# 34j/vr180-convert

Hardware: NVIDIA B200
Metric: SBS equirect output Mpix/s (higher is better)
Workload: dtype f64 coordinates / u8 fixed-point (INTER_BITS=5) sampling

## Files before the change

### vr180-convert_b200/csrc/api.cu

```cuda
#include <algorithm>
#include <mutex>
#include <new>
#include <string>
#include <vector>

#include "common.cuh"

namespace vr180 {

std::atomic<uint64_t> g_launches{0};
std::atomic<int> g_debug_frames_per_cta{0};
std::atomic<int> g_debug_tiled_flags{-1};
std::atomic<int> g_debug_max_frames_per_cta{0};
std::atomic<int> g_debug_stream_grid{0};
static thread_local std::string t_cuda_error;

void set_cuda_error(cudaError_t e, const char* where) {
    t_cuda_error = std::string(cudaGetErrorName(e)) + ": " + cudaGetErrorString(e) + " at " + where;
    cudaGetLastError();
}

const std::vector<int16_t>& host_table(int K);

}

using namespace vr180;

extern "C" {

int vr180_abi_version(void) { return VR180_ABI_VERSION; }

const char* vr180_status_string(int status) {
    switch (status) {
        case VR180_OK: return "ok";
        case VR180_ERR_INVALID_ARG: return "invalid argument";
        case VR180_ERR_UNSUPPORTED: return "unsupported configuration";
        case VR180_ERR_CUDA: return "CUDA error";
        case VR180_ERR_NO_DEVICE: return "no CUDA device";
        case VR180_ERR_CHAIN: return "malformed chain descriptor";
        case VR180_ERR_NOMEM: return "out of memory";
        default: return "unknown status";
    }
}

const char* vr180_last_cuda_error(void) { return t_cuda_error.c_str(); }

int vr180_device_info(int device, char* name, size_t name_len, int* sm_count, int* cc_major, int* cc_minor) {
    int n = 0;
    if (cudaGetDeviceCount(&n) != cudaSuccess) {
        cudaGetLastError();
        return 0;
    }
    if (device >= 0 && device < n) {
        cudaDeviceProp prop;
        if (cudaGetDeviceProperties(&prop, device) == cudaSuccess) {
            if (name && name_len) {
                strncpy(name, prop.name, name_len - 1);
                name[name_len - 1] = 0;
            }
            if (sm_count) *sm_count = prop.multiProcessorCount;
            if (cc_major) *cc_major = prop.major;
            if (cc_minor) *cc_minor = prop.minor;
        }
    }
    return n;
}

uint64_t vr180_launch_count(void) { return g_launches.load(std::memory_order_relaxed); }

int vr180_debug_weight_table(int K, int16_t* out) {
    if ((K != 4 && K != 8) || !out) return VR180_ERR_INVALID_ARG;
    const auto& t = host_table(K);
    memcpy(out, t.data(), t.size() * sizeof(int16_t));
    return VR180_OK;
}

int vr180_debug_set(int what, int value) {
    if (what == 0) return g_debug_frames_per_cta.exchange(value < 0 ? 0 : value);
    if (what == 1) return g_debug_tiled_flags.exchange(value);
    if (what == 2) return g_debug_max_frames_per_cta.exchange(value < 0 ? 0 : value);
    if (what == 3) return g_debug_stream_grid.exchange(value < 0 ? 0 : value);
    return VR180_ERR_INVALID_ARG;
}

int vr180_build_map(const vr180_chain_t* chain, int out_w, int out_h, float* xmap_dev, float* ymap_dev,
                    int64_t map_pitch, void* stream) {
    if (!chain || !xmap_dev || !ymap_dev || out_w <= 0 || out_h <= 0 || map_pitch < out_w) return VR180_ERR_INVALID_ARG;
    const int rc = validate_chain(chain);
    if (rc != VR180_OK) return rc;
    DeviceGuard g(xmap_dev);
    if (!g.ok) return VR180_ERR_INVALID_ARG;
    return launch_build_map(chain, out_w, out_h, xmap_dev, ymap_dev, map_pitch, (cudaStream_t)stream);
}

int vr180_pack_lut(const float* xmap_dev, const float* ymap_dev, int64_t map_pitch, int out_w, int out_h,
                   int32_t* fixed_dev, int64_t fixed_pitch, void* stream) {
    if (!xmap_dev || !ymap_dev || !fixed_dev || out_w <= 0 || out_h <= 0 || map_pitch < out_w || fixed_pitch < out_w)
        return VR180_ERR_INVALID_ARG;
    DeviceGuard g(fixed_dev);
    if (!g.ok) return VR180_ERR_INVALID_ARG;
    return launch_pack_lut(xmap_dev, ymap_dev, map_pitch, out_w, out_h, fixed_dev, fixed_pitch, (cudaStream_t)stream);
}

size_t vr180_packed_lut_bytes(int out_w, int out_h, int interpolation) {
    if (out_w <= 0 || out_h <= 0) return 0;
    return packed_lut_bytes(out_w, out_h, interpolation);
}

int vr180_pack_lut_tiles(const float* xmap_dev, const float* ymap_dev, int64_t map_pitch, int out_w, int out_h,
                         int interpolation, void* packed_dev, void* stream) {
    if (!xmap_dev || !ymap_dev || !packed_dev || out_w <= 0 || out_h <= 0 || map_pitch < out_w) return VR180_ERR_INVALID_ARG;
    if (packed_lut_bytes(out_w, out_h, interpolation) == 0) return VR180_ERR_UNSUPPORTED;
    DeviceGuard g(packed_dev);
    if (!g.ok) return VR180_ERR_INVALID_ARG;
    return launch_pack_lut_tiles(xmap_dev, ymap_dev, map_pitch, out_w, out_h, interpolation, packed_dev, (cudaStream_t)stream);
}

int vr180_remap(const vr180_remap_params_t* params, void* stream) {
    if (!params || !params->dst) return VR180_ERR_INVALID_ARG;
    DeviceGuard g(params->dst);
    if (!g.ok) return VR180_ERR_INVALID_ARG;
    return launch_remap(params, nullptr, (cudaStream_t)stream);
}

int vr180_remap_ex(const vr180_remap_params_t* params, const double border_scalar[4], void* stream) {
    if (!params || !params->dst) return VR180_ERR_INVALID_ARG;
    DeviceGuard g(params->dst);
    if (!g.ok) return VR180_ERR_INVALID_ARG;
    return launch_remap(params, border_scalar, (cudaStream_t)stream);
}

int vr180_anaglyph(const uint8_t* sbs_dev, int64_t sbs_pitch, int64_t sbs_frame_stride, int eye_w, int h, int n_frames,
                   uint8_t* out_dev, int64_t out_pitch, int64_t out_frame_stride, void* stream) {
    if (!sbs_dev || !out_dev || eye_w <= 0 || h <= 0 || n_frames < 0 || sbs_pitch < (int64_t)eye_w * 6 ||
        out_pitch < (int64_t)eye_w * 3)
        return VR180_ERR_INVALID_ARG;
    DeviceGuard g(out_dev);
    if (!g.ok) return VR180_ERR_INVALID_ARG;
    return launch_anaglyph(sbs_dev, sbs_pitch, sbs_frame_stride, eye_w, eye_w, h, n_frames, out_dev, out_pitch,
                           out_frame_stride, (cudaStream_t)stream);
}

int vr180_transform_points(const vr180_chain_t* chain, int64_t n, const double* x_dev, const double* y_dev,
                           double* out_x_dev, double* out_y_dev, double* out_v3_dev, void* stream) {
    if (!chain || n < 0 || !x_dev || !y_dev || (!out_v3_dev && !(out_x_dev && out_y_dev))) return VR180_ERR_INVALID_ARG;
    const int rc = validate_chain(chain);
    if (rc != VR180_OK) return rc;
    DeviceGuard g(x_dev);
    if (!g.ok) return VR180_ERR_INVALID_ARG;
    return launch_transform_points(chain, n, x_dev, y_dev, out_x_dev, out_y_dev, out_v3_dev, (cudaStream_t)stream);
}

int vr180_get_radius(const vr180_image_t* views, int n_views, int n_frames, double threshold, int32_t* transitions_dev,
                     double* radius_dev, void* stream) {
    if (!views || (!transitions_dev && !radius_dev)) return VR180_ERR_INVALID_ARG;
    DeviceGuard g(transitions_dev ? (const void*)transitions_dev : (const void*)radius_dev);
    if (!g.ok) return VR180_ERR_INVALID_ARG;
    return launch_get_radius(views, n_views, n_frames, threshold, transitions_dev, radius_dev, (cudaStream_t)stream);
}

int vr180_host_alloc(size_t bytes, void** out) {
    if (!out) return VR180_ERR_INVALID_ARG;
    VR180_CUDA(cudaHostAlloc(out, bytes ? bytes : 1, cudaHostAllocPortable));
    return VR180_OK;
// ... 18 lines not shown
```

### vr180-convert_b200/csrc/common.cuh

```cuda
#pragma once
#include <cuda_runtime.h>

#include <atomic>
#include <cstdint>
#include <cstdio>
#include <cstring>

#include "../../include/vr180_b200.h"

namespace vr180 {

extern std::atomic<uint64_t> g_launches;
extern std::atomic<int> g_debug_frames_per_cta;
extern std::atomic<int> g_debug_tiled_flags;
extern std::atomic<int> g_debug_max_frames_per_cta;
extern std::atomic<int> g_debug_stream_grid;
void set_cuda_error(cudaError_t e, const char* where);

#define VR180_CUDA(call)                                  \
    do {                                                  \
        cudaError_t e__ = (call);                         \
        if (e__ != cudaSuccess) {                         \
            ::vr180::set_cuda_error(e__, #call);          \
            return VR180_ERR_CUDA;                        \
        }                                                 \
    } while (0)

struct DeviceGuard {
    int prev = -1;
    int dev = -1;
    bool ok = false;
    explicit DeviceGuard(const void* ptr) {
        cudaPointerAttributes a;
        if (cudaPointerGetAttributes(&a, ptr) != cudaSuccess || a.type != cudaMemoryTypeDevice) {
            cudaGetLastError();
            return;
        }
        dev = a.device;
        if (cudaGetDevice(&prev) != cudaSuccess) return;
        if (prev != dev && cudaSetDevice(dev) != cudaSuccess) return;
        ok = true;
    }
    explicit DeviceGuard(int device) {
        dev = device;
        if (cudaGetDevice(&prev) != cudaSuccess) return;
        if (prev != dev && cudaSetDevice(dev) != cudaSuccess) return;
        ok = true;
    }
    ~DeviceGuard() {
        if (ok && prev != dev && prev >= 0) cudaSetDevice(prev);
    }
};

struct ViewArgs {
    const uint8_t* src;
    int rows, cols;
    long long pitch, frame_stride;
    int map_kind;
    int chain_idx;
    const float* xmap;
    const float* ymap;
    const int2* fixed;
    long long map_pitch;
    const double* radius_dev;
    int dst_x_offset;
    const void* packed;
};

struct RemapArgs {
    ViewArgs view[2];
    int n_views, n_frames, share_map;
    int W, H;
    int border_mode;
    uint8_t bv[4];
    int depth;
    uint8_t* dst;
    long long dst_pitch, dst_frame_stride;
    int frames_per_cta;
};

struct Remap16 {
    float cval[4];
    const float* ftab;
};

inline int depth_bytes(int depth) { return depth == VR180_DEPTH_16U ? 2 : 1; }

int launch_build_map(const vr180_chain_t* chain, int out_w, int out_h, float* xmap, float* ymap, int64_t pitch,
                     cudaStream_t st);
int launch_pack_lut(const float* xmap, const float* ymap, int64_t map_pitch, int out_w, int out_h, int32_t* fixed,
                    int64_t fixed_pitch, cudaStream_t st);
int launch_remap(const vr180_remap_params_t* p, const double* border_scalar, cudaStream_t st);
size_t packed_lut_bytes(int out_w, int out_h, int interp);
int launch_pack_lut_tiles(const float* xmap, const float* ymap, int64_t map_pitch, int out_w, int out_h, int interp,
                          void* packed, cudaStream_t st);
int launch_remap_tiled(const RemapArgs& a, int channels, int interp, const vr180_chain_t& c0, const vr180_chain_t& c1,
                       const short* weight_tab, cudaStream_t st);
int launch_get_radius(const vr180_image_t* views, int n_views, int n_frames, double threshold, int32_t* transitions,
                      double* radius, cudaStream_t st);
// ... 8 lines not shown
```

### vr180-convert_b200/csrc/tiled.cu

```cuda
#include "tiled.cuh"

namespace vr180 {
namespace tiled {

struct TileGeom {
    int rsel;
    int bx0, ry0;
    int x0, y0;
};

template <class M, int NV, bool DYN, int FR, bool SPLIT = false, bool VPAIR = false>
__device__ __forceinline__ void frame_loop(const RemapArgs& a, const TmaMaps& tm, int v_begin, int f0, int f1,
                                           const typename M::Pixel (&pc)[M::kPx], const TileGeom& tg, const int pitch,
                                           uint8_t* smem, int band, int cg, const DynRadius& dr,
                                           const double (&nx)[M::kPx], const double (&ny)[M::kPx], const short* tab) {
    static_assert(FR == 1 || !DYN, "a per-frame radius gives every frame its own rectangle");
    static_assert(M::kOutTiles / FR >= 2, "at least two out buffers of one item each");
    constexpr int kOutTileBytes = M::kTileH * kTileW * 3;
    constexpr int kOutItemBytes = FR * kOutTileBytes;
    constexpr int OB = M::kOutTiles / FR < kOutBufs ? M::kOutTiles / FR : kOutBufs;
    const int tid = threadIdx.x, lane = tid & 31, warp = tid >> 5;
    uint32_t s_stage = smem_u32(smem);
    asm volatile("" : "+r"(s_stage));
    const uint32_t s_full = s_stage + Lay<M>::kOffBar;
    const uint32_t s_ofull = s_full + 2 * kMaxStages * 8, s_oempty = s_ofull + kOutBufs * 8, s_out = s_stage + Lay<M>::kOffOut;

    int2* const s_org = reinterpret_cast<int2*>(smem + Lay<M>::kOffOrg);
    static_assert(!VPAIR || (SPLIT && FR == 2 && NV == 2 && !DYN), "an eye pair is two one-frame boxes of two views");
    const int n_items = VPAIR ? (f1 - f0) : ((f1 - f0 + FR - 1) / FR) * NV;
    const int rect_bytes = (M::kRowsMin + tg.rsel * kRowsStep) * pitch;
    const int stage_bytes = FR * rect_bytes;
    const int frame_pitch = SPLIT ? (rect_bytes + 127) & ~127 : rect_bytes;
    const int stage_stride = (FR * frame_pitch + 127) & ~127;
    static_assert(Lay<M>::kStageArea % 128 == 0 && Lay<M>::kStageArea / 128 <= 1024, "float quotient below");
    const int S = min(kMaxStages, (int)__fdividef((float)(Lay<M>::kStageArea / 128) + 0.5f, (float)(stage_stride >> 7)));

    if (warp == kSamplers / 32) {
        if (lane != 0) return;
        const CUtensorMap* const map0 = &tm.src[v_begin][(pitch - kPitchMin) / kPitchStep][tg.rsel];
        const int dst_x0 = (a.view[v_begin].dst_x_offset + tg.x0) * 3;
        const int dst_x1 = (a.view[v_begin + NV - 1].dst_x_offset + tg.x0) * 3;
        int p_item = 0, p_stage = 0;
        auto load = [&]() {
            const uint32_t bar = s_full + p_stage * 8;
            const int v = (NV == 2 && !VPAIR) ? (p_item & 1) : 0;
            const int f = VPAIR ? f0 + p_item : f0 + FR * ((NV == 2) ? (p_item >> 1) : p_item);
            int bx0 = tg.bx0, ry0 = tg.ry0;
            if (DYN) {
                const double rad = __ldg(dr.radius + f);
                if (rad == rad) {
                    int xlo, xhi, ylo, yhi;
                    dyn_range<M>(dr.ext[0], dr.ext[1], rad, dr.cx, xlo, xhi);
                    dyn_range<M>(dr.ext[2], dr.ext[3], rad, dr.cy, ylo, yhi);
                    const TileRect rc = tile_rect<M>(xlo, xhi, ylo, yhi);
                    bx0 = rc.bx0;
                    ry0 = rc.ry0;
                } else {
                    bx0 = ry0 = -(1 << 20);
                }
                s_org[p_stage] = make_int2(bx0, ry0);
            }
            mbar_expect_tx(bar, (uint32_t)stage_bytes);
            if (SPLIT) {
#pragma unroll
                for (int fr = 0; fr < FR; ++fr)
                    tma_load_3d(s_stage + p_stage * stage_stride + fr * frame_pitch,
                                map0 + (VPAIR ? fr : v) * (kWidths * kRowSizes), bx0, ry0, VPAIR ? f : f + fr, bar);
            } else {
                tma_load_3d(s_stage + p_stage * stage_stride, map0 + v * (kWidths * kRowSizes), bx0, ry0, f, bar);
            }
            ++p_item;
            if (++p_stage == S) p_stage = 0;
        };
        for (int n = 0; n < S && n < n_items; ++n) load();
        for (int n = 0; n < n_items; ++n) {
            const int o = n & (OB - 1);
            const int v = (NV == 2 && !VPAIR) ? (n & 1) : 0;
            const int f = VPAIR ? f0 + n : f0 + FR * ((NV == 2) ? (n >> 1) : n);
            mbar_wait(s_ofull + o * 8, (uint32_t)(n / OB) & 1u);
            if (n + S < n_items) load();
            if (SPLIT) {
#pragma unroll
                for (int fr = 0; fr < FR; ++fr)
                    tma_store_3d(&tm.dst, (VPAIR ? fr : v) ? dst_x1 : dst_x0, tg.y0, VPAIR ? f : f + fr,
                                 s_out + o * kOutItemBytes + fr * kOutTileBytes);
            } else {
                tma_store_3d(&tm.dst, v ? dst_x1 : dst_x0, tg.y0, f, s_out + o * kOutItemBytes);
            }
            bulk_commit();
            bulk_wait_read<0>();
            mbar_arrive(s_oempty + o * 8);
        }
        bulk_wait_read<0>();
        return;
    }

    const int sub = lane & 3;
    const uint32_t out_sel = sub == 0 ? 0x4210u : (sub == 1 ? 0x5421u : 0x6542u);
    const bool writer = sub != 3;
    constexpr int kOutStep = M::kRowPatch ? kTileW * 3 : 24;
    const int sw = band * (4 / M::kPx) + cg;
    uint32_t outp = s_out + (M::kRowPatch ? (M::kPx * sw) * (kTileW * 3) + (3 * (lane >> 2) + sub) * 4
                                          : (4 * band + (lane >> 3)) * (kTileW * 3) + M::kPx * cg * 24 +
                                                (3 * ((lane & 7) >> 2) + sub) * 4);
    uint32_t flags = (writer ? 1u : 0u) | (lane == 0 ? 2u : 0u);
    asm volatile("" : "+r"(outp), "+r"(flags));

    int st = 0;
    uint32_t ph = 0;
    typename M::Pixel cur[M::kPx];
    double cur_rad = CUDART_NAN;
    bool cur_have = false;
#pragma unroll
    for (int k = 0; k < M::kPx; ++k) cur[k] = pc[k];
    for (int n = 0; n < n_items; ++n) {
        mbar_wait(s_full + st * 8, ph);
        const uint32_t buf = s_stage + st * stage_stride;
        uint32_t res[FR][M::kPx];
        if (DYN) {
            const int f = f0 + ((NV == 2) ? (n >> 1) : n);
            const double rad = __ldg(dr.radius + f);
            if (!(rad == cur_rad)) {
                const int2 org = s_org[st];
                cur_have = rad == rad;
#pragma unroll
                for (int k = 0; k < M::kPx; ++k) {
                    const int qx = denorm_q<M>(nx[k], rad, dr.cx), qy = denorm_q<M>(ny[k], rad, dr.cy);
                    const int off = ((qy >> M::kShift) - M::kLo - org.y) * pitch + 3 * ((qx >> M::kShift) - M::kLo) - org.x;
                    M::set_offset(cur[k], off, cur_have);
                    M::weights(cur[k], qx & 31, qy & 31, tab);
                }
                cur_rad = rad;
            }
#pragma unroll
            for (int k = 0; k < M::kPx; ++k) {
                const uint32_t r = M::sample(buf, cur[k], (uint32_t)pitch);
                res[0][k] = cur_have ? r : 0u;
            }
        }
        uint32_t word[FR][M::kPx];
        if (!DYN && M::kInterp == VR180_INTER_LANCZOS4) {
#pragma unroll
            for (int k = 0; k < M::kPx; ++k) {
                uint32_t r[FR];
                sample_item<M, FR>(buf, (uint32_t)frame_pitch, pc[k], (uint32_t)pitch, r);
#pragma unroll
                for (int fr = 0; fr < FR; ++fr) res[fr][k] = r[fr];
            }
        }
#pragma unroll
        for (int fr = 0; fr < FR; ++fr) {
            if (!DYN && M::kInterp != VR180_INTER_LANCZOS4) {
#pragma unroll
                for (int k = 0; k < M::kPx; ++k) res[fr][k] = M::sample(buf + fr * frame_pitch, pc[k], (uint32_t)pitch);
            }
#pragma unroll
            for (int k = 0; k < M::kPx; ++k)
                word[fr][k] = __byte_perm(res[fr][k], __shfl_down_sync(0xffffffffu, res[fr][k], 1), out_sel);
        }
        const int o = n & (OB - 1);
        if (n >= OB) mbar_wait(s_oempty + o * 8, (uint32_t)(n / OB + 1) & 1u);
        if (flags & 1u) {
            const uint32_t ob = outp + o * kOutItemBytes;
#pragma unroll
            for (int fr = 0; fr < FR; ++fr)
#pragma unroll
                for (int k = 0; k < M::kPx; ++k) sts32(ob + fr * kOutTileBytes + k * kOutStep, word[fr][k]);
        }
        fence_proxy_async();
        __syncwarp();
        if (flags & 2u) mbar_arrive(s_ofull + o * 8);
        if (++st == S) { st = 0; ph ^= 1u; }
    }
}

template <class M, bool DYN, int FR>
__global__ void __launch_bounds__(kThreads, 4)
k_warp_tiled(const __grid_constant__ RemapArgs a, const __grid_constant__ vr180_chain_t chain0,
             const __grid_constant__ vr180_chain_t chain1, const __grid_constant__ TiledParams tp,
             const __grid_constant__ TmaMaps tm) {
    constexpr int kPx = M::kPx;
    constexpr int kChainUnroll = (FR == 1 && !DYN) ? kPx : 1;
    constexpr int kWarpsPerBand = 4 / kPx;
    extern __shared__ __align__(1024) uint8_t smem[];
    double* s_trig = reinterpret_cast<double*>(smem + Lay<M>::kOffTrig);
    int4* s_red = reinterpret_cast<int4*>(smem + Lay<M>::kOffRed);

    const int tid = threadIdx.x, lane = tid & 31, warp = tid >> 5;
    if (tid < 2 * kMaxStages + 2 * kOutBufs) {
        const uint32_t bars = smem_u32(smem + Lay<M>::kOffBar);
        const bool by_warps = (tid >= kMaxStages && tid < 2 * kMaxStages + kOutBufs);
        mbar_init(bars + tid * 8, by_warps ? kSamplers / 32 : 1);
        asm volatile("fence.mbarrier_init.release.cluster;" ::: "memory");
    }
    int* const s_cost = reinterpret_cast<int*>(smem + Lay<M>::kOffCost);
    if (tid < kPitchCands) s_cost[tid] = 0;
    const int tx = blockIdx.x, ty = blockIdx.y, tile = ty * tp.tiles_x + tx;
    const int x0 = tx * kTileW, y0 = ty * M::kTileH;
    const bool two_groups = !a.share_map && a.n_views == 2;
    const int g = two_groups ? (int)(blockIdx.z & 1u) : 0;
    const int chunk = two_groups ? (int)(blockIdx.z >> 1) : (int)blockIdx.z;
    const ViewArgs& mv = a.view[g];
    const int v_begin = g, v_end = a.share_map ? a.n_views : g + 1, nv = v_end - v_begin;
    const int f0 = chunk * a.frames_per_cta, f1 = min(a.n_frames, f0 + a.frames_per_cta);
    const bool sampler = warp < kSamplers / 32;
    const int sw = warp & (kSamplers / 32 - 1), band = sw / kWarpsPerBand, cg = sw % kWarpsPerBand;
    const int lx = M::kRowPatch ? lane : 8 * kPx * cg + (lane & 7), ly = M::kRowPatch ? kPx * sw : 4 * band + (lane >> 3);
    auto pcol = [&](int k) { return M::kRowPatch ? lx : lx + 8 * k; };
    auto prow = [&](int k) { return M::kRowPatch ? ly + k : ly; };
    const bool full_tile = (x0 + kTileW <= a.W) && (y0 + M::kTileH <= a.H);

    TileHdr hdr = {0, 0, 0, 0, 0};
    if (mv.map_kind != VR180_MAPSRC_ANALYTIC && mv.packed) hdr = decode_header(packed_header_raw(mv.packed, tile));
    const bool packed_tile = (hdr.flags & 1) != 0;

    int sx[kPx], sy[kPx];
    double nx[kPx], ny[kPx];
#pragma unroll
    for (int k = 0; k < kPx; ++k) {
        sx[k] = sy[k] = 0;
        nx[k] = ny[k] = 0.0;
    }
    constexpr bool dyn = DYN;
    if (mv.map_kind == VR180_MAPSRC_ANALYTIC) {
        const vr180_chain_t& ch = mv.chain_idx ? chain1 : chain0;
        const StdChain& sc = tp.std[mv.chain_idx ? 1 : 0];
        const bool fastc = sc.valid && sc.fast && !(tp.debug & 256);
        if (sc.valid || tp.sep_prefix) {
            if (tid < 64) {
                const bool is_row = tid >= 32;
                const int idx = tid & 31;
                const double* nm = ch.ops[0].p;
                const double c = (double)((is_row ? y0 : x0) + idx);
                const double n = mul_rn(__ddiv_rn(add_rn(c, -(is_row ? nm[1] : nm[0])), nm[2]), 2.0);
                double sv, cv;
                sincos(mul_rn(n, kHalfPi), &sv, &cv);
                if (fastc) {
                    std_tables(sc.R, sc.lat_is_y != 0, is_row, sv, cv, s_trig, s_trig + 128, idx);
                } else {
                    s_trig[(is_row ? 64 : 0) + idx] = sv;
                    s_trig[(is_row ? 96 : 32) + idx] = cv;
                }
            }
            __syncthreads();
            const bool lat_is_y = ch.ops[1].iparam != 0;
            auto seed = [&](int k, ChainState& s) {
                const double s_row = s_trig[64 + prow(k)], c_row = s_trig[96 + prow(k)];
                const double s_col = s_trig[pcol(k)], c_col = s_trig[32 + pcol(k)];
                s.mode = MODE_VEC3;
                s.x = s.y = s.r = s.ux = s.uy = 0.0;
                if (lat_is_y) {
                    s.vx = mul_rn(c_row, s_col);
                    s.vy = s_row;
                    s.vz = mul_rn(c_row, c_col);
                } else {
                    s.vx = s_col;
                    s.vy = mul_rn(c_col, s_row);
                    s.vz = mul_rn(c_col, c_row);
                }
            };
            if (!sampler) {
            } else if (fastc) {
                auto std_eval = [&](const StdChain& c) {
                    const bool x_fixed = M::kRowPatch ? !c.lat_is_y : (c.lat_is_y != 0);
                    const int fi = M::kRowPatch ? lx : ly;
                    const double* const ft = s_trig + (x_fixed ? 0 : 128) + fi;
                    const double f0 = ft[0], f1 = ft[32], f2 = ft[64], f3 = x_fixed ? ft[96] : 0.0;
#pragma unroll(kChainUnroll)
                    for (int k = 0; k < kPx; ++k) {
                        const int vi = M::kRowPatch ? prow(k) : pcol(k);
                        double vx, vy, vz;
                        if (x_fixed) {
                            vx = fma(f0, s_trig[128 + vi], f1); vy = fma(f0, s_trig[160 + vi], f2); vz = fma(f0, s_trig[192 + vi], f3);
                        } else {
                            const double sc_ = s_trig[vi];
                            vx = fma(sc_, f0, s_trig[32 + vi]); vy = fma(sc_, f1, s_trig[64 + vi]); vz = fma(sc_, f2, s_trig[96 + vi]);
                        }
                        double ox, oy;
                        int qx = 0, qy = 0;
                        if (dyn) {
                            std_pixel<true>(vx, vy, vz, c.poly, c.n_poly, c.den, ox, oy);
                        } else {
                            std_pixel<false>(vx, vy, vz, c.poly, c.n_poly, c.den, ox, oy);
                            qx = M::quant(__double2float_rn(ox));
// ... 144 lines not shown
            dr.ext[2] = fmin(dr.ext[2], s_ext[w * 4 + 2]);
            dr.ext[3] = fmax(dr.ext[3], s_ext[w * 4 + 3]);
        }
        const vr180_chain_t& ch = mv.chain_idx ? chain1 : chain0;
        dr.radius = mv.radius_dev;
        dr.cx = ch.ops[ch.n_ops - 1].p[2];
        dr.cy = ch.ops[ch.n_ops - 1].p[3];
        int ok = 1;
        for (int f = f0 + lane; f < f1; f += 32) {
            const double rad = __ldg(dr.radius + f);
            if (rad == rad) {
                int lo, hi, ylo, yhi;
                dyn_range<M>(dr.ext[0], dr.ext[1], rad, dr.cx, lo, hi);
                ok &= (lo > -32768) & (hi < 32767);
                dyn_range<M>(dr.ext[2], dr.ext[3], rad, dr.cy, ylo, yhi);
                ok &= (ylo > -32768) & (yhi < 32767);
                const TileRect rf = tile_rect<M>(lo, hi, ylo, yhi);
                dyn_wbytes = max(dyn_wbytes, rf.wbytes);
                dyn_nrows = max(dyn_nrows, rf.nrows);
                if (!tp.zero_border) ok &= inside_src(lo, hi, ylo, yhi) ? 1 : 0;
            } else if (!tp.zero_border) {
                ok = 0;
            }
        }
        dyn_wbytes = __reduce_max_sync(0xffffffffu, dyn_wbytes);
        dyn_nrows = __reduce_max_sync(0xffffffffu, dyn_nrows);
        ok = __all_sync(0xffffffffu, ok);
        fast = full_tile && ok && !nan_px && dyn_wbytes <= kPitchMax && box_rsel<M>(dyn_nrows) < kRowSizes &&
               stage_fits(M::kRowsMin + box_rsel<M>(dyn_nrows) * kRowsStep, max(dyn_wbytes, kPitchMin));
    }

    if (!fast) {
        if (sampler) {
#pragma unroll
            for (int k = 0; k < kPx; ++k) {
                const int i = x0 + pcol(k), j = y0 + prow(k);
                if (i < a.W && j < a.H) {
                    for (int f = f0; f < f1; ++f) {
                        int qx = sx[k], qy = sy[k];
                        if (dynr) {
                            const double rad = __ldg(dr.radius + f);
                            qx = denorm_q<M>(nx[k], rad, dr.cx);
                            qy = denorm_q<M>(ny[k], rad, dr.cy);
                        }
                        gather_pixel<M>(a, f, i, j, v_begin, v_end, qx, qy, tp.tab);
                    }
                }
            }
        }
        return;
    }

    int pitch = max(dynr ? dyn_wbytes : rc.wbytes, kPitchMin);
    if (!dynr && (f1 - f0) * nv >= 8) {
        if (sampler) pitch_costs<M>(sx[0], sy[0], rc, pitch, lane, s_cost);
        __syncthreads();
        pitch = pick_pitch(s_cost, pitch, rc.box_rows, [&](int pe) { return stage_fits(rc.box_rows, pe); });
    }

    typename M::Pixel pc[kPx];
#pragma unroll
    for (int k = 0; k < kPx; ++k) {
        const int ix = sx[k] >> M::kShift, iy = sy[k] >> M::kShift;
        const int off = (iy - M::kLo - rc.ry0) * pitch + 3 * (ix - M::kLo) - rc.bx0;
        M::set_offset(pc[k], off, true);
        if (sampler && !dynr) M::weights(pc[k], sx[k] & 31, sy[k] & 31, tp.tab);
    }
    if constexpr (M::kWeightSmem != 0) {
        if (!dynr && sampler) {
            uint8_t* slot = smem + Lay<M>::kOffW + tid * 16;
#pragma unroll
            for (int ky = 0; ky < 8; ++ky)
                *reinterpret_cast<uint4*>(slot + ky * (kSamplers * 16)) = __ldg(reinterpret_cast<const uint4*>(pc[0].w) + ky);
            pc[0].ws = smem_u32(slot);
        }
    }
    TileGeom tg;
    tg.rsel = dynr ? box_rsel<M>(dyn_nrows) : rc.rsel;
    tg.bx0 = rc.bx0;
    tg.ry0 = rc.ry0;
    tg.x0 = x0;
    tg.y0 = y0;
    if (DYN && dynr) {
        if (nv == 2) frame_loop<M, 2, DYN, 1>(a, tm, v_begin, f0, f1, pc, tg, pitch, smem, band, cg, dr, nx, ny, tp.tab);
        else         frame_loop<M, 1, DYN, 1>(a, tm, v_begin, f0, f1, pc, tg, pitch, smem, band, cg, dr, nx, ny, tp.tab);
    } else {
        if constexpr (!DYN && FR == 1) {
            if (nv == 2) frame_loop<M, 2, false, 2, true, true>(a, tm, v_begin, f0, f1, pc, tg, pitch, smem, band, cg, dr, nx, ny, tp.tab);
            else         frame_loop<M, 1, false, 1, false>(a, tm, v_begin, f0, f1, pc, tg, pitch, smem, band, cg, dr, nx, ny, tp.tab);
        } else {
            if (nv == 2) frame_loop<M, 2, false, FR, DYN>(a, tm, v_begin, f0, f1, pc, tg, pitch, smem, band, cg, dr, nx, ny, tp.tab);
            else         frame_loop<M, 1, false, FR, DYN>(a, tm, v_begin, f0, f1, pc, tg, pitch, smem, band, cg, dr, nx, ny, tp.tab);
        }
    }
}

template <class M>
__global__ void __launch_bounds__(kSamplers) k_pack_tiles(const float* __restrict__ xmap, const float* __restrict__ ymap,
                                                         long long map_pitch, int W, int H, int tiles_x, int n_tiles,
                                                         void* __restrict__ packed) {
    constexpr int kPx = M::kPx;
    __shared__ int4 s_red[kSamplers / 32];
    __shared__ int s_cost[kPitchCands];
    const int tid = threadIdx.x, lane = tid & 31, sw = tid >> 5;
    const int tx = blockIdx.x % tiles_x, ty = blockIdx.x / tiles_x;
    const int x0 = tx * kTileW, y0 = ty * M::kTileH;
    const bool full_tile = (x0 + kTileW <= W) && (y0 + M::kTileH <= H);
    if (tid < kPitchCands) s_cost[tid] = 0;
    int sx[kPx], sy[kPx];
#pragma unroll
    for (int k = 0; k < kPx; ++k) {
        const int i = x0 + lane, j = y0 + kPx * sw + k;
        sx[k] = sy[k] = (int)0x80000000;
        if (i < W && j < H) {
            sx[k] = M::quant(__ldg(xmap + (long long)j * map_pitch + i));
            sy[k] = M::quant(__ldg(ymap + (long long)j * map_pitch + i));
        }
    }
    block_box_store<M>(sx, sy, s_red, sw, lane == 0);
    __syncthreads();
    const int4 box = block_box_load(s_red, lane);
    const int mnx = box.x, mxx = box.y, mny = box.z, mxy = box.w;
    const bool ok = full_tile && mnx > -32768 && mny > -32768 && mxx < 32767 && mxy < 32767 && mxx - mnx <= 255 &&
                    mxy - mny <= 255;
    const TileRect rc = tile_rect<M>(mnx, mxx, mny, mxy);
    const bool stageable = ok && rc.wbytes <= kPitchMax && rc.rsel < kRowSizes;
    const int pitch0 = max(rc.wbytes, kPitchMin);
    if (stageable) pitch_costs<M>(sx[0], sy[0], rc, pitch0, lane, s_cost);
    __syncthreads();
    const int pitch = !stageable ? kPitchMin : pick_pitch(s_cost, pitch0, rc.box_rows, [&](int pe) {
        return pe == pitch0 || rc.box_rows * pe <= kStreamSlotBytes<M>;
    });
    const int widx = (pitch - kPitchMin) / kPitchStep;
    if (tid == 0) {
        int4 h;
        h.x = (mnx & 0xffff) | (mxx << 16);
        h.y = (mny & 0xffff) | (mxy << 16);
        h.z = (ok ? kHdrPackable : 0) | (stageable ? kHdrStageable : 0) |
              (stageable && rc.box_rows * pitch <= kStreamSlotBytes<M> ? kHdrFitsSlot : 0) | (widx << 8) | (rc.rsel << 12);
        h.w = 0;
        reinterpret_cast<int4*>(packed)[blockIdx.x] = h;
    }
    uint32_t* ent = reinterpret_cast<uint32_t*>(static_cast<uint8_t*>(packed) + packed_entries_offset(n_tiles)) +
                    ((size_t)blockIdx.x * kSamplers + tid) * kPx;
#pragma unroll
    for (int k = 0; k < kPx; ++k) {
        const int ix = sat16(sx[k] >> M::kShift), iy = sat16(sy[k] >> M::kShift);
        const uint32_t fx = M::kShift ? (uint32_t)(sx[k] & 31) : 0u, fy = M::kShift ? (uint32_t)(sy[k] & 31) : 0u;
        ent[k] = ok ? ((uint32_t)(ix - mnx) | ((uint32_t)(iy - mny) << 8) | (fx << 16) | (fy << 21)) : 0u;
    }
}

}

static int tile_height_of(int interp) {
    return interp == VR180_INTER_LINEAR || interp == VR180_INTER_NEAREST ? tiled::LinearP::kTileH
           : interp == VR180_INTER_CUBIC                                  ? tiled::Cubic::kTileH
           : interp == VR180_INTER_LANCZOS4                               ? tiled::Lanczos4::kTileH
                                                                          : 0;
}

size_t packed_lut_bytes(int out_w, int out_h, int interp) {
    const int th = tile_height_of(interp);
    if (!th) return 0;
    const long long n_tiles = (long long)((out_w + tiled::kTileW - 1) / tiled::kTileW) * ((out_h + th - 1) / th);
    return tiled::packed_entries_offset(n_tiles) + (size_t)n_tiles * tiled::kTileW * th * 4;
}

int launch_pack_lut_tiles(const float* xmap, const float* ymap, int64_t map_pitch, int W, int H, int interp, void* packed,
                          cudaStream_t st) {
    using namespace tiled;
    const int th = tile_height_of(interp);
    if (!th) return VR180_ERR_UNSUPPORTED;
    const int tiles_x = (W + kTileW - 1) / kTileW, tiles_y = (H + th - 1) / th;
    const long long n_tiles = (long long)tiles_x * tiles_y;
    if (n_tiles > 0x7fffffffLL) return VR180_ERR_UNSUPPORTED;
// ... 124 lines not shown
    key.dst_pitch = a0.dst_pitch;
    key.dst_fs = a0.dst_frame_stride;
    struct Entry {
        Key key;
        TmaMaps tm;
        uint64_t stamp;
    };
    constexpr size_t kCacheEntries = 8;
    static thread_local std::vector<Entry> cache;
    static thread_local uint64_t clock_ = 0;
    Entry* hit = nullptr;
    for (Entry& e : cache)
        if (memcmp(&key, &e.key, sizeof(key)) == 0) hit = &e;
    if (!hit) {
        if (cache.size() < kCacheEntries) {
            cache.emplace_back();
            hit = &cache.back();
        } else {
            hit = &cache[0];
            for (Entry& e : cache)
                if (e.stamp < hit->stamp) hit = &e;
        }
        memset(&hit->key, 0xff, sizeof(hit->key));
        TmaMaps& t = hit->tm;
        memset(&t, 0, sizeof(t));
        for (int v = 0; v < a0.n_views; ++v) {
            const ViewArgs& vw = a0.view[v];
            for (int w = 0; w < kWidths; ++w)
                for (int r = 0; r < kRowSizes; ++r)
                    if (!encode_u8_3d(&t.src[v][w][r], vw.src, (long long)vw.cols * 3, vw.rows, a0.n_frames, vw.pitch,
                                      vw.frame_stride, kPitchMin + w * kPitchStep, rows_min + r * kRowsStep, fr))
                        return nullptr;
        }
        if (a0.n_views == 1) memcpy(&t.src[1], &t.src[0], sizeof(t.src[0]));
        if (!encode_u8_3d(&t.dst, a0.dst, a0.dst_pitch, a0.H, a0.n_frames, a0.dst_pitch, a0.dst_frame_stride, kTileW * 3,
                          tile_h, fr))
            return nullptr;
        hit->key = key;
    }
    hit->stamp = ++clock_;
    return &hit->tm;
}

template <class M, bool DYN, int FR>
static int launch_mode(const RemapArgs& a0, const vr180_chain_t& c0, const vr180_chain_t& c1, const short* tab,
                       cudaStream_t st) {
    using namespace tiled;
    const int n_groups = a0.share_map ? 1 : a0.n_views;
    const TmaMaps* tmp = tma_maps_for(a0, M::kInterp, M::kRowsMin, M::kTileH, DYN ? 1 : FR);
    if (!tmp) return VR180_ERR_UNSUPPORTED;
    const TmaMaps& tm = *tmp;

    int dev = 0;
    const int rc = max_dyn_smem_once<k_warp_tiled<M, DYN, FR>>(Lay<M>::kSmemBytes, dev);
    if (rc != VR180_OK) return rc;

    RemapArgs a = a0;
    TiledParams tp;
    memset(&tp, 0, sizeof(tp));
    const int tiles_x = (a.W + kTileW - 1) / kTileW, tiles_y = (a.H + M::kTileH - 1) / M::kTileH;
    tp.tiles_x = tiles_x;
    tp.n_tiles = tiles_x * tiles_y;
    tp.tab = tab;
    tp.zero_border = zero_border(a);
    tp.debug = tiled_debug_flags();
    const long long tiles = (long long)tiles_x * tiles_y * n_groups;
    int fpc = frames_per_cta(tiles, a.n_frames, a.share_map ? a.n_views : 1);
    fpc = (fpc + FR - 1) / FR * FR;
    a.frames_per_cta = fpc;
    const int chunks = (a.n_frames + fpc - 1) / fpc;
    if (n_groups > 2 || chunks * n_groups > 65535 || tiles_y > 65535 || tiles_x * (long long)tiles_y > 0x7fffffffLL)
        return VR180_ERR_UNSUPPORTED;
    auto is_sep = [](const vr180_chain_t& c) {
        return c.n_ops >= 2 && c.ops[0].code == VR180_OP_NORMALIZE && c.ops[1].code == VR180_OP_EQUIRECT_ENC;
    };
    tp.sep_prefix = 1;
    for (int g = 0; g < n_groups; ++g) {
        if (a.view[g].map_kind != VR180_MAPSRC_ANALYTIC) continue;
        const vr180_chain_t& c = a.view[g].chain_idx ? c1 : c0;
        if (!is_sep(c)) tp.sep_prefix = 0;
        match_std_chain(c, tp.std[a.view[g].chain_idx ? 1 : 0]);
    }
    dim3 grid((unsigned)tiles_x, (unsigned)tiles_y, (unsigned)(n_groups * chunks));
    k_warp_tiled<M, DYN, FR><<<grid, kThreads, Lay<M>::kSmemBytes, st>>>(a, c0, c1, tp, tm);
    g_launches.fetch_add(1, std::memory_order_relaxed);
    VR180_CUDA(cudaGetLastError());
    return VR180_OK;
}

template <class M>
static int launch_tiled(const RemapArgs& a0, const vr180_chain_t& c0, const vr180_chain_t& c1, const short* tab, bool dyn,
                        int fpc, cudaStream_t st) {
    if constexpr (M::kInterp == VR180_INTER_CUBIC) {
        if (fpc >= 8) return dyn ? launch_mode<M, true, 4>(a0, c0, c1, tab, st) : launch_mode<M, false, 4>(a0, c0, c1, tab, st);
    }
    if (fpc >= 2) return dyn ? launch_mode<M, true, 2>(a0, c0, c1, tab, st) : launch_mode<M, false, 2>(a0, c0, c1, tab, st);
    return dyn ? launch_mode<M, true, 1>(a0, c0, c1, tab, st) : launch_mode<M, false, 1>(a0, c0, c1, tab, st);
}

int launch_remap_tiled(const RemapArgs& a0, int channels, int interp, const vr180_chain_t& c0, const vr180_chain_t& c1,
                       const short* weight_tab, cudaStream_t st) {
    if (channels != 3 || a0.depth != VR180_DEPTH_8U) return VR180_ERR_UNSUPPORTED;
    if (interp != VR180_INTER_NEAREST && interp != VR180_INTER_LINEAR && interp != VR180_INTER_CUBIC &&
        interp != VR180_INTER_LANCZOS4)
        return VR180_ERR_UNSUPPORTED;
    if (interp == VR180_INTER_NEAREST)
        for (int v = 0; v < a0.n_views; ++v)
            if (a0.view[v].map_kind == VR180_MAPSRC_FIXED) return VR180_ERR_UNSUPPORTED;
    const int n_groups = a0.share_map ? 1 : a0.n_views;
    for (int v = 0; v < a0.n_views; ++v) {
        const ViewArgs& vw = a0.view[v];
        if (((uintptr_t)vw.src & 15) || (vw.pitch & 15) || (vw.frame_stride & 15) || vw.pitch < (long long)vw.cols * 3)
            return VR180_ERR_UNSUPPORTED;
        if (a0.n_frames > 1 && vw.frame_stride < vw.pitch * vw.rows) return VR180_ERR_UNSUPPORTED;
        if (vw.rows != a0.view[0].rows || vw.cols != a0.view[0].cols) return VR180_ERR_UNSUPPORTED;
        if ((vw.dst_x_offset * 3) & 15) return VR180_ERR_UNSUPPORTED;
    }
    if (((uintptr_t)a0.dst & 15) || (a0.dst_pitch & 15) || (a0.dst_frame_stride & 15)) return VR180_ERR_UNSUPPORTED;
    if (a0.n_frames > 1 && a0.dst_frame_stride < a0.dst_pitch * a0.H) return VR180_ERR_UNSUPPORTED;
    int n_dyn = 0;
    for (int g = 0; g < n_groups; ++g)
        n_dyn += (a0.view[g].map_kind == VR180_MAPSRC_ANALYTIC && a0.view[g].radius_dev) ? 1 : 0;
    if (n_dyn != 0 && n_dyn != n_groups) return VR180_ERR_UNSUPPORTED;
    const bool dyn = n_dyn != 0;
    const int kStreamMaxItems = a0.share_map ? 20 : 16;
    {
        bool all_packed = !dyn;
        for (int g = 0; g < n_groups; ++g) all_packed = all_packed && a0.view[g].packed != nullptr;
        const int dbg = tiled_debug_flags();
        const int items = a0.n_frames * (a0.share_map ? a0.n_views : 1);
        const bool tab_ok = (interp != VR180_INTER_CUBIC && interp != VR180_INTER_LANCZOS4) || weight_tab != nullptr;
        if (all_packed && tab_ok && !(dbg & 4) && ((dbg & 2) || items <= kStreamMaxItems) &&
            g_debug_frames_per_cta.load(std::memory_order_relaxed) <= 0) {
            const int rc = launch_remap_stream(a0, interp, weight_tab, st);
            if (rc != VR180_ERR_UNSUPPORTED) return rc;
        }
    }
    const int tile_h = tile_height_of(interp);
    const long long tiles = (long long)((a0.W + tiled::kTileW - 1) / tiled::kTileW) * ((a0.H + tile_h - 1) / tile_h) * n_groups;
    const int fpc = frames_per_cta(tiles, a0.n_frames, a0.share_map ? a0.n_views : 1);
    if (interp == VR180_INTER_NEAREST) return launch_tiled<tiled::Nearest>(a0, c0, c1, nullptr, dyn, fpc, st);
    if (interp == VR180_INTER_LINEAR) return launch_tiled<tiled::LinearP>(a0, c0, c1, nullptr, dyn, fpc, st);
    if (!weight_tab) return VR180_ERR_UNSUPPORTED;
    if (interp == VR180_INTER_LANCZOS4) return launch_tiled<tiled::Lanczos4>(a0, c0, c1, weight_tab, dyn, fpc, st);
    return launch_tiled<tiled::Cubic>(a0, c0, c1, weight_tab, dyn, fpc, st);
}

}
```

### vr180-convert_b200/csrc/tiled.cuh

```cuda
#pragma once
#include <cuda.h>

#include <cmath>
#include <cstdlib>
#include <mutex>
#include <type_traits>
#include <vector>

#include "chain_fast.cuh"
#include "common.cuh"
#include "sampler.cuh"

namespace vr180 {
namespace tiled {

constexpr int kTileW = 32;
constexpr int kSamplers = 256;
constexpr int kThreads = kSamplers + 32;
constexpr int kMaxStages = 8;
constexpr int kRowsStep = 4, kRowSizes = 9;
constexpr int kPitchMin = 96, kPitchMax = 256, kPitchStep = 16;
constexpr int kWidths = (kPitchMax - kPitchMin) / kPitchStep + 1;
constexpr int kPitchCands = 4;
constexpr int kStageAreaDefault = 40960;
constexpr int kOutBufs = 4;
template <class M>
struct Lay {
    static constexpr int kStageArea = M::kStageArea;
    static constexpr int kOutArea = M::kOutTiles * M::kTileH * kTileW * 3;
    static constexpr int kOffOut = kStageArea;
    static constexpr int kOffTrig = kOffOut + kOutArea;
    static constexpr int kOffRed = kOffTrig + 7 * 32 * 8;
    static constexpr int kOffBar = kOffRed + 8 * 4 * 4;
    static constexpr int kOffOrg = kOffBar + (2 * kMaxStages + 2 * kOutBufs) * 8;
    static constexpr int kOffExt = kOffOrg + kMaxStages * 8;
    static constexpr int kOffCost = kOffExt + 8 * 4 * 8;
    static constexpr int kOffW = (kOffCost + 16 + 15) & ~15;
    static constexpr int kSmemBytes = kOffW + M::kWeightSmem;
};

template <class M>
constexpr int kStreamSlotBytes = (M::kStageArea / 3) & ~127;

struct StdChain {
    int valid, lat_is_y, has_rot, n_poly;
    int fast, pad_;
    double norm[3];
    double R[9];
    double poly[VR180_MAX_OP_PARAMS];
    double den[4];
};

struct TiledParams {
    int tiles_x;
    int n_tiles;
    int sep_prefix;
    int debug;
    int zero_border;
    const short* tab;
    StdChain std[2];
};

struct alignas(64) TmaMaps {
    CUtensorMap src[2][kWidths][kRowSizes];
    CUtensorMap dst;
};

struct PackedHdr {
    short mnx, mxx, mny, mxy;
    int flags;
    int pad;
};
constexpr int kHdrPackable = 1;
constexpr int kHdrStageable = 2;
constexpr int kHdrFitsSlot = 4;
static_assert(sizeof(PackedHdr) == 16, "PackedHdr is one 128-bit load");
__host__ __device__ inline size_t packed_entries_offset(long long n_tiles) { return ((size_t)n_tiles * 16 + 255) & ~(size_t)255; }
__device__ __forceinline__ int4 packed_header_raw(const void* packed, int tile) {
    return __ldg(reinterpret_cast<const int4*>(packed) + tile);
}
struct TileHdr {
    int mnx, mxx, mny, mxy, flags;
};
__device__ __forceinline__ TileHdr decode_header(const int4& v) {
    return {(short)(v.x & 0xffff), v.x >> 16, (short)(v.y & 0xffff), v.y >> 16, v.z};
}
template <class M>
__device__ __forceinline__ void load_packed_entries(const void* packed, int n_tiles, int tile, int tid, uint32_t (&e)[M::kPx]) {
    const uint32_t* ent = reinterpret_cast<const uint32_t*>(static_cast<const uint8_t*>(packed) + packed_entries_offset(n_tiles)) +
                          ((size_t)tile * kSamplers + tid) * M::kPx;
    if constexpr (M::kPx == 4) {
        const uint4 v = __ldg(reinterpret_cast<const uint4*>(ent));
        e[0] = v.x; e[1] = v.y; e[2] = v.z; e[3] = v.w;
    } else if constexpr (M::kPx == 2) {
        const uint2 v = __ldg(reinterpret_cast<const uint2*>(ent));
        e[0] = v.x; e[1] = v.y;
    } else {
        e[0] = __ldg(ent);
    }
}
template <class M>
__device__ __forceinline__ int2 unpack_entry(int hdr_mnx, int hdr_mny, uint32_t e) {
    return make_int2(((hdr_mnx + (int)(e & 255u)) << M::kShift) | (int)((e >> 16) & 31u),
                     ((hdr_mny + (int)((e >> 8) & 255u)) << M::kShift) | (int)((e >> 21) & 31u));
}

__device__ __forceinline__ uint32_t smem_u32(const void* p) { return (uint32_t)__cvta_generic_to_shared(p); }

__device__ __forceinline__ void mbar_init(uint32_t bar, uint32_t count) {
    asm volatile("mbarrier.init.shared::cta.b64 [%0], %1;" ::"r"(bar), "r"(count) : "memory");
}
__device__ __forceinline__ void mbar_expect_tx(uint32_t bar, uint32_t bytes) {
    asm volatile("mbarrier.arrive.expect_tx.shared::cta.b64 _, [%0], %1;" ::"r"(bar), "r"(bytes) : "memory");
}
__device__ __forceinline__ void mbar_arrive(uint32_t bar) {
    asm volatile("mbarrier.arrive.shared::cta.b64 _, [%0];" ::"r"(bar) : "memory");
}
constexpr uint32_t kSuspendNs = 4000;
__device__ __forceinline__ void mbar_wait(uint32_t bar, uint32_t parity) {
    asm volatile(
        "{\n\t.reg .pred p;\n\t"
        "WAIT_%=:\n\t"
        "mbarrier.try_wait.parity.shared::cta.b64 p, [%0], %1, %2;\n\t"
        "@p bra DONE_%=;\n\t"
        "bra WAIT_%=;\n\t"
        "DONE_%=:\n\t}" ::"r"(bar), "r"(parity), "r"(kSuspendNs)
        : "memory");
}
__device__ __forceinline__ void fence_proxy_async() { asm volatile("fence.proxy.async.shared::cta;" ::: "memory"); }
__device__ __forceinline__ void tma_load_3d(uint32_t dst, const CUtensorMap* map, int x, int y, int z, uint32_t bar) {
    asm volatile(
        "cp.async.bulk.tensor.3d.shared::cluster.global.tile.mbarrier::complete_tx::bytes [%0], [%1, {%2, %3, %4}], [%5];" ::
            "r"(dst), "l"(map), "r"(x), "r"(y), "r"(z), "r"(bar)
        : "memory");
}
__device__ __forceinline__ void tma_store_3d(const CUtensorMap* map, int x, int y, int z, uint32_t src) {
    asm volatile("cp.async.bulk.tensor.3d.global.shared::cta.tile.bulk_group [%0, {%1, %2, %3}], [%4];" ::"l"(map), "r"(x),
                 "r"(y), "r"(z), "r"(src)
                 : "memory");
}
__device__ __forceinline__ void bulk_commit() { asm volatile("cp.async.bulk.commit_group;" ::: "memory"); }
template <int N>
__device__ __forceinline__ void bulk_wait_read() {
// ... 362 lines not shown
```

Measured before the change: 719,900.

## Make linear FR=2 tiled remap kernel persistent with ring state carried across tiles

For the linear, non-dynamic, two-frame tiled path, the grid becomes 4×SM-count persistent CTAs that loop over tile/group/chunk work items. The mbarrier ring phase and out-buffer index are carried across tiles so the TMA stage and output rings continue without re-initialisation. Reduction and cost scratch in shared memory are double-buffered by parity so consecutive tiles do not collide. The aim is to cut CTA launch and tail overhead and let one tile's pipeline overlap the next, at the cost of more complex phase tracking and a small shared-memory increase.

```diff
diff --git a/vr180-convert_b200/csrc/api.cu b/vr180-convert_b200/csrc/api.cu
--- a/vr180-convert_b200/csrc/api.cu
+++ b/vr180-convert_b200/csrc/api.cu
@@ -13,6 +13,7 @@
 std::atomic<int> g_debug_tiled_flags{-1};
 std::atomic<int> g_debug_max_frames_per_cta{0};
 std::atomic<int> g_debug_stream_grid{0};
+std::atomic<int> g_debug_tiled_grid{0};
 static thread_local std::string t_cuda_error;
 
 void set_cuda_error(cudaError_t e, const char* where) {
@@ -80,6 +81,7 @@
     if (what == 1) return g_debug_tiled_flags.exchange(value);
     if (what == 2) return g_debug_max_frames_per_cta.exchange(value < 0 ? 0 : value);
     if (what == 3) return g_debug_stream_grid.exchange(value < 0 ? 0 : value);
+    if (what == 4) return g_debug_tiled_grid.exchange(value < 0 ? 0 : value);
     return VR180_ERR_INVALID_ARG;
 }
 
diff --git a/vr180-convert_b200/csrc/common.cuh b/vr180-convert_b200/csrc/common.cuh
--- a/vr180-convert_b200/csrc/common.cuh
+++ b/vr180-convert_b200/csrc/common.cuh
@@ -15,6 +15,7 @@
 extern std::atomic<int> g_debug_tiled_flags;
 extern std::atomic<int> g_debug_max_frames_per_cta;
 extern std::atomic<int> g_debug_stream_grid;
+extern std::atomic<int> g_debug_tiled_grid;
 void set_cuda_error(cudaError_t e, const char* where);
 
 #define VR180_CUDA(call)                                  \
diff --git a/vr180-convert_b200/csrc/tiled.cu b/vr180-convert_b200/csrc/tiled.cu
--- a/vr180-convert_b200/csrc/tiled.cu
+++ b/vr180-convert_b200/csrc/tiled.cu
@@ -9,11 +9,17 @@
     int x0, y0;
 };
 
-template <class M, int NV, bool DYN, int FR, bool SPLIT = false, bool VPAIR = false>
+struct RingState {
+    int items;
+    uint32_t full_ph;
+};
+
+template <class M, int NV, bool DYN, int FR, bool SPLIT = false, bool VPAIR = false, bool PERSIST = false>
 __device__ __forceinline__ void frame_loop(const RemapArgs& a, const TmaMaps& tm, int v_begin, int f0, int f1,
                                            const typename M::Pixel (&pc)[M::kPx], const TileGeom& tg, const int pitch,
                                            uint8_t* smem, int band, int cg, const DynRadius& dr,
-                                           const double (&nx)[M::kPx], const double (&ny)[M::kPx], const short* tab) {
+                                           const double (&nx)[M::kPx], const double (&ny)[M::kPx], const short* tab,
+                                           RingState& rs) {
     static_assert(FR == 1 || !DYN, "a per-frame radius gives every frame its own rectangle");
     static_assert(M::kOutTiles / FR >= 2, "at least two out buffers of one item each");
     constexpr int kOutTileBytes = M::kTileH * kTileW * 3;
@@ -34,6 +40,8 @@
     const int stage_stride = (FR * frame_pitch + 127) & ~127;
     static_assert(Lay<M>::kStageArea % 128 == 0 && Lay<M>::kStageArea / 128 <= 1024, "float quotient below");
     const int S = min(kMaxStages, (int)__fdividef((float)(Lay<M>::kStageArea / 128) + 0.5f, (float)(stage_stride >> 7)));
+    const int nb = PERSIST ? rs.items : 0;
+    if (PERSIST) rs.items = nb + n_items;
 
     if (warp == kSamplers / 32) {
         if (lane != 0) return;
@@ -74,10 +82,10 @@
         };
         for (int n = 0; n < S && n < n_items; ++n) load();
         for (int n = 0; n < n_items; ++n) {
-            const int o = n & (OB - 1);
+            const int o = (nb + n) & (OB - 1);
             const int v = (NV == 2 && !VPAIR) ? (n & 1) : 0;
             const int f = VPAIR ? f0 + n : f0 + FR * ((NV == 2) ? (n >> 1) : n);
-            mbar_wait(s_ofull + o * 8, (uint32_t)(n / OB) & 1u);
+            mbar_wait(s_ofull + o * 8, (uint32_t)((nb + n) / OB) & 1u);
             if (n + S < n_items) load();
             if (SPLIT) {
 #pragma unroll
@@ -113,8 +121,10 @@
     bool cur_have = false;
 #pragma unroll
     for (int k = 0; k < M::kPx; ++k) cur[k] = pc[k];
+    uint32_t full_ph = PERSIST ? rs.full_ph : 0u;
     for (int n = 0; n < n_items; ++n) {
-        mbar_wait(s_full + st * 8, ph);
+        if (PERSIST) mbar_wait(s_full + st * 8, (full_ph >> st) & 1u);
+        else mbar_wait(s_full + st * 8, ph);
         const uint32_t buf = s_stage + st * stage_stride;
         uint32_t res[FR][M::kPx];
         if (DYN) {
@@ -158,8 +168,8 @@
             for (int k = 0; k < M::kPx; ++k)
                 word[fr][k] = __byte_perm(res[fr][k], __shfl_down_sync(0xffffffffu, res[fr][k], 1), out_sel);
         }
-        const int o = n & (OB - 1);
-        if (n >= OB) mbar_wait(s_oempty + o * 8, (uint32_t)(n / OB + 1) & 1u);
+        const int o = (nb + n) & (OB - 1);
+        if (nb + n >= OB) mbar_wait(s_oempty + o * 8, (uint32_t)((nb + n) / OB + 1) & 1u);
         if (flags & 1u) {
             const uint32_t ob = outp + o * kOutItemBytes;
 #pragma unroll
@@ -170,8 +180,10 @@
         fence_proxy_async();
         __syncwarp();
         if (flags & 2u) mbar_arrive(s_ofull + o * 8);
+        if (PERSIST) full_ph ^= 1u << st;
         if (++st == S) { st = 0; ph ^= 1u; }
     }
+    if (PERSIST) rs.full_ph = full_ph;
 }
 
 template <class M, bool DYN, int FR>
@@ -184,7 +196,7 @@
     constexpr int kWarpsPerBand = 4 / kPx;
     extern __shared__ __align__(1024) uint8_t smem[];
     double* s_trig = reinterpret_cast<double*>(smem + Lay<M>::kOffTrig);
-    int4* s_red = reinterpret_cast<int4*>(smem + Lay<M>::kOffRed);
+    int4* const s_red2 = reinterpret_cast<int4*>(smem + Lay<M>::kOffRed);
 
     const int tid = threadIdx.x, lane = tid & 31, warp = tid >> 5;
     if (tid < 2 * kMaxStages + 2 * kOutBufs) {
@@ -193,13 +205,17 @@
         mbar_init(bars + tid * 8, by_warps ? kSamplers / 32 : 1);
         asm volatile("fence.mbarrier_init.release.cluster;" ::: "memory");
     }
-    int* const s_cost = reinterpret_cast<int*>(smem + Lay<M>::kOffCost);
+    constexpr bool kPersist = std::is_same<M, LinearP>::value && !DYN && FR == 2;
+    RingState rs = {0, 0u};
+    auto tile_body = [&](const int tx, const int ty, const int z, const int par) {
+    int4* const s_red = s_red2 + par * (kSamplers / 32);
+    int* const s_cost = reinterpret_cast<int*>(smem + Lay<M>::kOffCost) + par * kPitchCands;
     if (tid < kPitchCands) s_cost[tid] = 0;
-    const int tx = blockIdx.x, ty = blockIdx.y, tile = ty * tp.tiles_x + tx;
+    const int tile = ty * tp.tiles_x + tx;
     const int x0 = tx * kTileW, y0 = ty * M::kTileH;
     const bool two_groups = !a.share_map && a.n_views == 2;
-    const int g = two_groups ? (int)(blockIdx.z & 1u) : 0;
-    const int chunk = two_groups ? (int)(blockIdx.z >> 1) : (int)blockIdx.z;
+    const int g = two_groups ? (z & 1) : 0;
+    const int chunk = two_groups ? (z >> 1) : z;
     const ViewArgs& mv = a.view[g];
     const int v_begin = g, v_end = a.share_map ? a.n_views : g + 1, nv = v_end - v_begin;
     const int f0 = chunk * a.frames_per_cta, f1 = min(a.n_frames, f0 + a.frames_per_cta);
@@ -510,16 +526,27 @@
     tg.x0 = x0;
     tg.y0 = y0;
     if (DYN && dynr) {
-        if (nv == 2) frame_loop<M, 2, DYN, 1>(a, tm, v_begin, f0, f1, pc, tg, pitch, smem, band, cg, dr, nx, ny, tp.tab);
-        else         frame_loop<M, 1, DYN, 1>(a, tm, v_begin, f0, f1, pc, tg, pitch, smem, band, cg, dr, nx, ny, tp.tab);
+        if (nv == 2) frame_loop<M, 2, DYN, 1>(a, tm, v_begin, f0, f1, pc, tg, pitch, smem, band, cg, dr, nx, ny, tp.tab, rs);
+        else         frame_loop<M, 1, DYN, 1>(a, tm, v_begin, f0, f1, pc, tg, pitch, smem, band, cg, dr, nx, ny, tp.tab, rs);
     } else {
         if constexpr (!DYN && FR == 1) {
-            if (nv == 2) frame_loop<M, 2, false, 2, true, true>(a, tm, v_begin, f0, f1, pc, tg, pitch, smem, band, cg, dr, nx, ny, tp.tab);
-            else         frame_loop<M, 1, false, 1, false>(a, tm, v_begin, f0, f1, pc, tg, pitch, smem, band, cg, dr, nx, ny, tp.tab);
+            if (nv == 2) frame_loop<M, 2, false, 2, true, true>(a, tm, v_begin, f0, f1, pc, tg, pitch, smem, band, cg, dr, nx, ny, tp.tab, rs);
+            else         frame_loop<M, 1, false, 1, false>(a, tm, v_begin, f0, f1, pc, tg, pitch, smem, band, cg, dr, nx, ny, tp.tab, rs);
         } else {
-            if (nv == 2) frame_loop<M, 2, false, FR, DYN>(a, tm, v_begin, f0, f1, pc, tg, pitch, smem, band, cg, dr, nx, ny, tp.tab);
-            else         frame_loop<M, 1, false, FR, DYN>(a, tm, v_begin, f0, f1, pc, tg, pitch, smem, band, cg, dr, nx, ny, tp.tab);
-        }
+            if (nv == 2) frame_loop<M, 2, false, FR, DYN, false, kPersist>(a, tm, v_begin, f0, f1, pc, tg, pitch, smem, band, cg, dr, nx, ny, tp.tab, rs);
+            else         frame_loop<M, 1, false, FR, DYN, false, kPersist>(a, tm, v_begin, f0, f1, pc, tg, pitch, smem, band, cg, dr, nx, ny, tp.tab, rs);
+        }
+    }
+    };
+
+    if constexpr (kPersist) {
+        int par = 0;
+        for (int w = blockIdx.x; w < tp.n_work; w += gridDim.x, par ^= 1) {
+            const int txy = w % tp.n_tiles, ty = txy / tp.tiles_x;
+            tile_body(txy - ty * tp.tiles_x, ty, w / tp.n_tiles, par);
+        }
+    } else {
+        tile_body((int)blockIdx.x, (int)blockIdx.y, (int)blockIdx.z, 0);
     }
 }
 
@@ -810,6 +837,15 @@
         match_std_chain(c, tp.std[a.view[g].chain_idx ? 1 : 0]);
     }
     dim3 grid((unsigned)tiles_x, (unsigned)tiles_y, (unsigned)(n_groups * chunks));
+    if (std::is_same<M, LinearP>::value && !DYN && FR == 2) {
+        if ((long long)tp.n_tiles * n_groups * chunks > 0x7fffffffLL) return VR180_ERR_UNSUPPORTED;
+        tp.n_work = tp.n_tiles * n_groups * chunks;
+        int sms = 0;
+        VR180_CUDA(cudaDeviceGetAttribute(&sms, cudaDevAttrMultiProcessorCount, dev));
+        const int forced = g_debug_tiled_grid.load(std::memory_order_relaxed);
+        const int ctas = forced > 0 ? forced : 4 * sms;
+        grid = dim3((unsigned)(ctas < tp.n_work ? ctas : tp.n_work));
+    }
     k_warp_tiled<M, DYN, FR><<<grid, kThreads, Lay<M>::kSmemBytes, st>>>(a, c0, c1, tp, tm);
     g_launches.fetch_add(1, std::memory_order_relaxed);
     VR180_CUDA(cudaGetLastError());
diff --git a/vr180-convert_b200/csrc/tiled.cuh b/vr180-convert_b200/csrc/tiled.cuh
--- a/vr180-convert_b200/csrc/tiled.cuh
+++ b/vr180-convert_b200/csrc/tiled.cuh
@@ -31,11 +31,11 @@
     static constexpr int kOffOut = kStageArea;
     static constexpr int kOffTrig = kOffOut + kOutArea;
     static constexpr int kOffRed = kOffTrig + 7 * 32 * 8;
-    static constexpr int kOffBar = kOffRed + 8 * 4 * 4;
+    static constexpr int kOffBar = kOffRed + 2 * 8 * 4 * 4;
     static constexpr int kOffOrg = kOffBar + (2 * kMaxStages + 2 * kOutBufs) * 8;
     static constexpr int kOffExt = kOffOrg + kMaxStages * 8;
     static constexpr int kOffCost = kOffExt + 8 * 4 * 8;
-    static constexpr int kOffW = (kOffCost + 16 + 15) & ~15;
+    static constexpr int kOffW = (kOffCost + 2 * 4 * kPitchCands + 15) & ~15;
     static constexpr int kSmemBytes = kOffW + M::kWeightSmem;
 };
 
@@ -59,6 +59,7 @@
     int zero_border;
     const short* tab;
     StdChain std[2];
+    int n_work;
 };
 
 struct alignas(64) TmaMaps {
```

Measured after the change: 409,000 (median of 6 runs). -43.2%, worse.
